# asharakeh/bayes-od-rc

Hardware: AMD Instinct MI355X
Metric: images/sec at N=10 MC samples, 512x512; per-anchor covariance latency (higher is better)
Workload: dtype bf16; 1 GPU; ResNet-50 RetinaNet + covar head, N=10 MC-dropout, 512x512, full BayesOD pipeline (forward+posterior+soft-NMS+cluster-fuse); global_batch=512, mc_samples=10, anchors=49104, parallelism=one GPU (no exchange; N > 1: image-sharded, one RCCL gather/step), visible_gpus=1, gpu_max_hw_queues=4

## Files before the change

### bayes-od-rc_amd/csrc/conv_igemm.hip

```cpp
#include "kernels.h"
#include "philox.h"
#include <cstdlib>
#include <string>
#include <type_traits>

typedef __attribute__((ext_vector_type(8))) short bf16x8;
typedef __attribute__((ext_vector_type(16))) float f32x16;
typedef __attribute__((ext_vector_type(4))) float f32x4;
typedef __attribute__((ext_vector_type(4))) unsigned int u32x4;
typedef __attribute__((ext_vector_type(8))) _Float16 f16x8;
typedef __attribute__((ext_vector_type(8))) int i32x8;
typedef __attribute__((ext_vector_type(6))) int i32x6;
typedef __attribute__((ext_vector_type(4))) int i32x4;
typedef __attribute__((ext_vector_type(16))) float f32x16v;
__device__ __forceinline__ i32x8 mx_cat(const bf16x8& p0, const bf16x8& p1) {
    return __builtin_shufflevector(__builtin_bit_cast(i32x4, p0), __builtin_bit_cast(i32x4, p1), 0, 1, 2, 3, 4, 5, 6, 7);
}

#define GLOBAL_PTR(p) ((const __attribute__((address_space(1))) void*)(p))
#define LDS_PTR(p) ((__attribute__((address_space(3))) void*)(p))

__device__ __forceinline__ float bf16_to_f32(uint32_t v) { return __uint_as_float(v << 16); }
__device__ __forceinline__ uint32_t f32_to_bf16(float f) {
    uint32_t u = __float_as_uint(f);
// ... 2201 lines not shown
                uint4 r;
                r.x = relu_bf16x2(v.x); r.y = relu_bf16x2(v.y); r.z = relu_bf16x2(v.z); r.w = relu_bf16x2(v.w);
                *reinterpret_cast<uint4*>(reinterpret_cast<uint16_t*>(G.out_relu) + e) = r;
            }
        }
        phase_stamp<ABL>(tstamp, 5);
        if constexpr (ABL == 90) { if (threadIdx.x == 0) atomicAdd(&g_phase_cycles[14], __builtin_amdgcn_s_memrealtime() - treal); }
        if (n + 1 < fan) __syncthreads();
    }
}

template <int BC, int BP, int WC, int WP, int ABL, bool XR, bool SPLIT = false>
__global__ __launch_bounds__(64 * WC * WP, (ABL == 10 ? (BC == 64 ? 3 : 2) : 1)) void conv_igemm_kernel(const ConvArgs a) {
    extern __shared__ __attribute__((aligned(16))) char smem[];
    int bx = blockIdx.x, by = blockIdx.y, gz = blockIdx.z;
    const int ny_tiles = a.cout_pad / BC;
    if (!XR && gridDim.y == 1 && ny_tiles > 1) {
        const int nx = (a.M + BP - 1) / BP, q = nx >> 3, r = nx & 7, xcd = bx & 7, slot = bx >> 3;
        const int pj = slot / ny_tiles;
        by = slot - pj * ny_tiles;
        if (pj >= q + (xcd < r ? 1 : 0)) return;
        bx = (xcd < r ? xcd * (q + 1) : r * (q + 1) + (xcd - r) * q) + pj;
    } else {
        const int nb = gridDim.x, q = nb >> 3, r = nb & 7, xcd = bx & 7, idx = bx >> 3;
        bx = (xcd < r ? xcd * (q + 1) : r * (q + 1) + (xcd - r) * q) + idx;
    }
    if (gridDim.z == 1 && a.groups > 1 && a.ksplit <= 1) {
        if (a.fan_chunk > 0) {
            const int nxt = (a.M + BP - 1) / BP, T = a.fan_chunk, per = T * a.groups;
            const int c = bx / per, w = bx - c * per, here = min(T, nxt - c * T);
// ... 305 lines not shown
    ConvArgs a_local = a_in;
    if ((a_local.flags & CONV_DROPOUT) && a_local.drop_threshold == 0) a_local.flags &= ~CONV_DROPOUT;
    static const bool res_register = getenv("BOD_RES_REGISTER") && atoi(getenv("BOD_RES_REGISTER")) == 1;
    if (res_register && a_local.variant == 0 && !a_local.xreuse && !a_local.split && a_local.ksplit <= 1) a_local.variant = 82;
    static const int nt_stores = getenv("BOD_NT_STORES") ? atoi(getenv("BOD_NT_STORES")) : 4;
    if (!(a_local.flags & CONV_OUT_F32) && !a_local.split && a_local.ksplit <= 1 &&
        (((nt_stores & 1) && !a_local.xreuse) || ((nt_stores & 2) && a_local.xreuse) || ((nt_stores & 4) && a_local.xreuse && a_local.fan_count > 1)))
        a_local.flags |= CONV_NT_OUT;
    if (a_local.mx && (((nt_stores & 8) && a_local.fan_count <= 1) || ((nt_stores & 16) && a_local.fan_count > 1))) a_local.flags |= CONV_NT_OUT;
    {
        static const int fan_chunk = getenv("BOD_FAN_CHUNK") ? atoi(getenv("BOD_FAN_CHUNK")) : 16;
        a_local.fan_chunk = (a_local.fan_count > 1 && a_local.groups > 1 && !a_local.mx && !a_local.split) ? fan_chunk : 0;
    }
    const ConvArgs& a = a_local;
    if (a.M <= 0) return hipSuccess;
    if (a.cin % 64 != 0 || a.cout_pad % 64 != 0) return hipErrorInvalidValue;
    if (a.mx) {
        if ((a.mx < 1 || a.mx > 3) || !a.split || a.xreuse != 2 || a.cout_pad != 256 || a.cin != 512 || a.taps != 9 || a.KW != 3 || !a.ext || a.M % 256 != 0 ||
            (a.flags & CONV_OUT_F32) || a.ksplit > 1 || (a.variant != 0 && a.variant != 90 && a.variant != 91) || a.groups < 1 || a.groups > 3)
            return hipErrorInvalidValue;
        for (int g = 0; g < a.groups; ++g)
            if (a.g[g].res || a.g[g].out_relu || a.g[g].ch_w2 || a.g[g].ch_w3 || (a.g[g].w2 && (a.g[g].out_hx || a.fan_count > 1))) return hipErrorInvalidValue;
#ifndef BOD_DEV_MX_ONLY
        if (a.variant == 90 && a.mx == 1) return launch_mx<11>(a, s);
        if (a.variant == 91 && a.mx == 1) return launch_mx<12>(a, s);
#endif
#ifdef BOD_DEV_MX_ONLY
        return a.mx == 1 ? launch_mx<1>(a, s) : hipErrorInvalidValue;
#else
        if (a.mx == 3) return a.variant == 0 ? launch_mx<3>(a, s) : hipErrorInvalidValue;
// ... 40 lines not shown
    }
    if (a.split) {
        if (a.xreuse) {
            if (!(big && a.cout_pad == 256 && a.taps == 9 && a.KW == 3 && a.ext && a.M % 256 == 0) || (a.flags & CONV_OUT_F32)) return hipErrorInvalidValue;
            return launch_cfg<256, 256, 2, 4, 0, true, true>(a, s);
        }
        if (big) return launch_cfg<256, 256, 2, 4, 0, false, true>(a, s);
        if (a.cout_pad % 128 == 0) return launch_cfg<128, 128, 2, 2, 0, false, true>(a, s);
        return launch_cfg<64, 128, 1, 4, 0, false, true>(a, s);
    }
    const int variant = a.variant;
    if (a.xreuse) {
        if (!(big && a.cout_pad == 256 && a.taps == 9 && a.KW == 3 && a.ext && a.M % 256 == 0)) return hipErrorInvalidValue;
        for (int g = 0; g < a.groups; ++g) if (a.g[g].res || a.g[g].out_relu) return hipErrorInvalidValue;
        if (a.flags & CONV_OUT_F32) return hipErrorInvalidValue;
        if (a.xreuse != 2 || a.variant == 81) return launch_cfg<256, 256, 2, 4, 81, true>(a, s);
        if (a.variant == 1) return launch_cfg<256, 256, 2, 4, 1, true>(a, s);
        if (a.variant == 2) return launch_cfg<256, 256, 2, 4, 2, true>(a, s);
        if (a.variant == 4) return launch_cfg<256, 256, 2, 4, 4, true>(a, s);
        if (a.variant == 30) return launch_cfg<256, 256, 2, 4, 30, true>(a, s);
        if (a.variant == 90) return launch_cfg<256, 256, 2, 4, 90, true>(a, s);
        if (a.variant == 96) return launch_xr_persistent<0>(a, s);
        if (a.variant == 31) return launch_cfg<256, 256, 2, 4, 31, true>(a, s);
        if (a.variant != 0 && a.variant != 83) return hipErrorInvalidValue;
        if (a.fan_count > 1) return launch_cfg<256, 256, 2, 4, 5, true>(a, s);
        if (a.plane_h > 0 && !(a.flags & CONV_DROPOUT) && a.variant == 0) return launch_cfg<256, 256, 2, 4, 6, true>(a, s);
        static const bool old_loop = getenv("BOD_TOWER_MIDBAR") && atoi(getenv("BOD_TOWER_MIDBAR")) == 0;
        if (old_loop && a.variant == 0) return launch_cfg<256, 256, 2, 4, 9, true>(a, s);
        return launch_cfg<256, 256, 2, 4, 0, true>(a, s);
    }
// ... 21 lines not shown
```

### bayes-od-rc_amd/csrc/engine.hip

```cpp
#include "../../include/bayesod.h"
#include "kernels.h"

#include <algorithm>
#include <atomic>
#include <cmath>
#include <condition_variable>
#include <deque>
#include <functional>
#include <mutex>
#include <thread>
#include <tuple>
#include <cstdarg>
#include <cstdio>
#include <cstring>
#include <map>
#include <memory>
#include <string>
#include <vector>
#include <dlfcn.h>

namespace {

constexpr float BN_EPS = 1e-3f;

thread_local std::string g_create_error;

struct HostTensor { std::vector<int64_t> shape; std::vector<float> data; };

struct Plane {
    char* d = nullptr;
    int64_t base = 0;
    int64_t bstride = 0;
    int h = 0, w = 0, C = 0, pitch = 0;
};

struct PackedConv { char* w = nullptr; float* bias = nullptr; int cout = 0, cout_pad = 0, taps = 0, kw = 0, cin = 0; };

struct Op {
    enum Kind { STEM, POOL, CONV } kind;
    ConvArgs conv;
    bool is_head3x3 = false;
    double flops = 0;
    std::string name;
    std::string wname[3], bnname[3];
    bool same_geom = false;
    int flavour = 0;
    int head[3] = {-1, -1, -1};
    bool hx_pyramid = false;
};
enum { FLAVOUR_BOTH = 0, FLAVOUR_RAW = 1, FLAVOUR_AGG = 2 };

uint16_t f2bf(float f) {
    uint32_t u; std::memcpy(&u, &f, 4);
    u += 0x7FFFu + ((u >> 16) & 1u);
// ... 185 lines not shown
    char* stem_out = nullptr;
    int es = 2;
    bool split = false;
    char* pyr_hx = nullptr;
    int pyr_fmt = 1;
    int plan_mx = 0;
    int mx = 0;
    Plane pyramid;
    char* head_act[3][2] = {{nullptr}};
    char* head_act_t[3][4] = {{nullptr}};
    float* raw[3] = {nullptr};
    float* agg[3] = {nullptr};
    bool agg_plan = false;
    bool plan_fused_out = false, plan_xreuse = false, plan_xreuse0 = false;
    bool raw_valid = false, agg_valid = false;
    uint64_t last_seed = 0; uint32_t last_first_image = 0;
    std::map<std::string, RowEnt*> tables;
    struct XrTable { RowEnt* rows = nullptr; int2* ext = nullptr; int m = 0; };
    std::map<std::string, XrTable> xr_tables;
    std::vector<Op> ops;
    const float* cur_images = nullptr;

    float* d_anchors = nullptr;
    PostBuffers pb{};
    float* nms_scores = nullptr; int32_t* nms_begin = nullptr;
    int32_t* nms_sel_s[2] = {nullptr, nullptr}; int32_t* nms_nsel_s[2] = {nullptr, nullptr};
    float* out_scores_s[2] = {nullptr, nullptr}; float* out_means_s[2] = {nullptr, nullptr};
    float* out_covs_s[2] = {nullptr, nullptr}; float* out_counts_s[2] = {nullptr, nullptr};
    int32_t* nms_sel = nullptr; int32_t* nms_nsel = nullptr;
    float* out_scores = nullptr; float* out_means = nullptr; float* out_covs = nullptr; float* out_counts = nullptr;
// ... 625 lines not shown
        if (rc == 1) return h->fail(BOD_ERR_INVALID_ARG, "aggregated tiling: no pixel fits a tile (N = %d)", N);
        if (rc == 2) return h->fail(BOD_ERR_INVALID_ARG, "aggregated tiling: extended rows out of order");
        m2a = (int)tiled.size();
        BODCHK(h->dalloc(&d2a, tiled.size(), false));
        BODCHK(h->dalloc(&dexta, ext.size(), false));
        HIPCHK(h, hipMemcpyAsync(d2a, tiled.data(), tiled.size() * sizeof(RowEnt), hipMemcpyHostToDevice, h->stream));
        HIPCHK(h, hipMemcpyAsync(dexta, ext.data(), ext.size() * sizeof(int2), hipMemcpyHostToDevice, h->stream));
        HIPCHK(h, hipStreamSynchronize(h->stream));
        const size_t BA = (size_t)B * h->A;
        BODCHK(h->dalloc(&h->agg[0], BA * c.num_classes));
        BODCHK(h->dalloc(&h->agg[1], BA * 16));
        if (c.has_covar_head) BODCHK(h->dalloc(&h->agg[2], BA * 10));
    } else {
        BODCHK(ensure_raw(h));
    }
    h->agg_plan = agg; h->plan_fused_out = fuse_out; h->plan_xreuse = xreuse; h->plan_xreuse0 = xreuse0; h->plan_mx = mx_plan ? mxf : 0;
    int hfmt[3] = {mxf, mxf, mxf};
    if (mxf == 2) { const char* e = getenv("BOD_MX4_BOX_HX"); if (e && atoi(e) != 0) hfmt[1] = 1; }
    if (mxf == 1) { static const bool cls_h4 = [] { const char* e = getenv("BOD_MX_CLS_H4"); return !e || atoi(e) != 0; }(); if (cls_h4) hfmt[0] = 2; }
    const bool mixed = mx_plan && hfmt[0] != hfmt[1];
    const int pyr_fmt = mixed ? 1 : mxf;
    h->pyr_fmt = pyr_fmt;
    for (int layer = 0; layer < 4; ++layer)
    for (int fpass = 0; fpass < 2; ++fpass)
    for (int part = 0; part < 2; ++part)
    for (int flav = (agg && layer >= 2) ? FLAVOUR_RAW : FLAVOUR_BOTH; flav <= ((agg && layer >= 2) ? FLAVOUR_AGG : FLAVOUR_BOTH); ++flav) {
        static const bool split_on = [] { const char* e = getenv("BOD_SPLIT_AGG_LAUNCH"); return !e || atoi(e) != 0; }();
        const bool split_launch = agg && layer >= 2 && split_on;
        if (fpass == 1 && (!mixed || layer == 0)) continue;
        const int lfmt = !mx_plan ? 0 : layer == 0 ? pyr_fmt : mixed ? (fpass == 0 ? 2 : 1) : mxf;
        if (!split_launch && part == 1) continue;
        if (split_launch && part == 0 && flav == FLAVOUR_AGG) continue;
        const bool both = split_launch && part == 0;
        Op op; op.kind = Op::CONV; op.is_head3x3 = true; op.flavour = both ? FLAVOUR_BOTH : flav;
        int g = 0; PackedConv pc0{};
        double fused_flops = 0;
        for (int hd = 0; hd < nheads; ++hd) {
            if (layer >= kHeadConvs[hd]) continue;
            if (split_launch && (part == 1) != (layer == kHeadConvs[hd] - 1)) continue;
            if (mixed && layer > 0 && hfmt[hd] != lfmt) continue;
            PackedConv pc;
            BODCHK(pack_conv(h, std::string(kHeadPrefix[hd]) + "_" + std::to_string(layer), "", 128, &pc, (mx_plan && (layer > 0 || mx_l0)) ? lfmt : 0));
// ... 8 lines not shown
            cg.out_hx = (mx_plan && layer < kHeadConvs[hd] - 1) ? hfmt[hd] : 0;
            if (fuse_out && layer == kHeadConvs[hd] - 1) {
                PackedConv po;
                BODCHK(pack_conv(h, kHeadPrefix[hd], "", 32, &po));
                if (po.cin != 256 || po.cout != out_ch[hd] || po.taps != 1)
                    return h->fail(BOD_ERR_INVALID_ARG, "head output conv %s must be 1x1 256->%d (got %d->%d)", kHeadPrefix[hd], out_ch[hd], po.cin, po.cout);
                cg.w2 = po.w; cg.bias2 = po.bias; cg.out2 = h->raw[hd]; cg.cout2 = po.cout; cg.out2_cstride = out_ch[hd];
                op.head[g] = hd;
                if (flav == FLAVOUR_AGG) {
                    cg.out2 = nullptr;
                    cg.agg_kind = hd == 0 ? AGG_CLS : hd == 1 ? AGG_BOX : AGG_COV;
                    cg.agg_n = N; cg.agg_P = h->P; cg.agg_C = c.num_classes; cg.agg_out = h->agg[hd]; cg.anchors = h->d_anchors;
                }
                fused_flops += 2.0 * ((double)B * N * h->P) * 256.0 * out_ch[hd];
            }
            op.conv.g[g] = cg;
            if (g == 0) pc0 = pc;
            ++g;
        }
        if (g == 0) continue;
        const int M = layer == 0 ? B * h->P : B * N * h->P;
        ConvArgs a = base_args(pc0, layer == 0 ? d1 : d2, M, 256, 256);
        for (int q = 0; q < g; ++q) a.g[q] = op.conv.g[q];
        a.groups = g;
        a.flags = CONV_RELU | (mc ? CONV_DROPOUT : 0);
        a.fan_count = layer == 0 ? N : 1;
        a.fan_stride = (int32_t)h->Ppad;
        a.drop_threshold = thr; a.drop_scale = dscale;
        a.mx = mx_plan ? ((layer == 0 && !mx_l0) ? 2 : (lfmt == 2 ? 3 : 1)) : 0;
        op.hx_pyramid = mx_l0 && layer == 0;
// ... 2 lines not shown
            static const int tower_loader = getenv("BOD_TOWER_LOADER") ? atoi(getenv("BOD_TOWER_LOADER")) : 0;
            a.mx_loader = mx_plan ? mx_loader : ((h->es == 2 && layer > 0) ? tower_loader : 0);
        }
        if (xreuse0 && layer == 0) { a.rows = d1x; a.M = m1x; a.ext = dext1; a.xreuse = 2; }
        if (xreuse && layer > 0) {
            a.rows = d2x; a.M = m2x; a.ext = dext;
            if (agg && layer >= 2 && !(split_launch && part == 0)) { a.rows = d2a; a.M = m2a; a.ext = dexta; }
            a.xreuse = 2;
        }
        op.conv = a;
        op.flops = 2.0 * M * 256.0 * 2304.0 * g + fused_flops;
        op.name = "head_tower_layer_" + std::to_string(layer) + (both ? "" : flav == FLAVOUR_AGG ? "(aggregating)" : flav == FLAVOUR_RAW ? "(raw)" : "");
        op.same_geom = N == 1;
        h->ops.push_back(op);
    }
    for (int hd = 0; hd < nheads && !fuse_out; ++hd) {
        PackedConv pc;
        BODCHK(pack_conv(h, kHeadPrefix[hd], "", 64, &pc));
        if (pc.cin != 256 || pc.cout != out_ch[hd] || pc.taps != 1)
            return h->fail(BOD_ERR_INVALID_ARG, "head output conv %s must be 1x1 256->%d (got %d->%d)", kHeadPrefix[hd], out_ch[hd], pc.cin, pc.cout);
        Op op; op.kind = Op::CONV;
        ConvArgs a = base_args(pc, d3, B * N * h->P, 256, out_ch[hd]);
        a.g[0] = ConvGroup{train_mode ? h->head_act_t[hd][kHeadConvs[hd] - 1] : h->head_act[hd][(kHeadConvs[hd] - 1) & 1], pc.w, pc.bias, h->raw[hd], nullptr, nullptr, 0, 0, nullptr, nullptr, nullptr, 0, 0};
        a.flags = CONV_OUT_F32;
        op.conv = a;
        op.flops = 2.0 * a.M * pc.cout * 256.0;
        op.name = kHeadPrefix[hd]; op.wname[0] = kHeadPrefix[hd];
        h->ops.push_back(op);
    }
    if (h->splitk_elems) {
// ... 125 lines not shown
    h->ov_dirty = false;
    return BOD_OK;
}

bod_status run_forward(bod_context* h, const float* dev_images, uint64_t seed, uint32_t first_image, int flavour = FLAVOUR_RAW,
                       bool only_flavoured = false, bool overlapped = false) {
    const bod_config& c = h->cfg;
    if (flavour == FLAVOUR_RAW && !only_flavoured) BODCHK(ensure_raw(h));
    const bool ov = overlapped && h->overlap_mode != 0 && !only_flavoured;
    hipStream_t fs = ov ? h->front : h->stream;
    int par = 0;
    if (ov) {
        par = h->fwd_parity; h->fwd_parity ^= 1;
        if (h->l0_pending[par]) { HIPCHK(h, hipStreamWaitEvent(fs, h->ev_l0_done[par], 0)); h->l0_pending[par] = false; }
    }
    if (!only_flavoured) h->pyr_last = par;
    const int cus_front = h->n_cu;
    const int cus_back = h->n_cu;
    static const int trace_call = getenv("BOD_TRACE_OPS") ? atoi(getenv("BOD_TRACE_OPS")) : 0;
    static int call_no = 0;
    const bool trace = trace_call > 0 && ++call_no == trace_call && !ov;
    std::vector<hipEvent_t> tev;
    if (trace) {
        tev.resize(h->ops.size() + 1);
        for (hipEvent_t& e : tev) HIPCHK(h, hipEventCreate(&e));
        HIPCHK(h, hipEventRecord(tev[0], h->stream));
    }
    size_t op_i = 0;
    bool stem_pool_fused = false;
    std::string cur_stage;
    struct StageCloser { std::string& s; ~StageCloser() { if (!s.empty()) markers().pop(); } } stage_closer{cur_stage};
// ... 18 lines not shown
            }
        }
        switch (op.kind) {
            case Op::STEM: {
                const Op* pool = op_i < h->ops.size() && h->ops[op_i].kind == Op::POOL ? &h->ops[op_i] : nullptr;
                static const bool split_fused = [] { const char* e = getenv("BOD_STEM_SPLIT_FUSED"); return !e || atoi(e) != 0; }();
                stem_pool_fused = pool && !h->train && (h->split ? split_fused : h->es == 2) && !trace &&
                                  stem_pool_fused_applies(dev_images, c.batch, c.image_w, h->sw, is_front ? cus_front : cus_back);
                if (stem_pool_fused)
                    HIPCHK(h, launch_stem_pool_fused(dev_images, h->stem_w, h->stem_b, pool->conv.g[0].out, h->split ? 1 : 0, c.batch, c.image_h,
                                                     c.image_w, h->sh, h->sw, h->ph, h->pw, h->pw + 2, (h->ph + 2) * (h->pw + 2), st));
                else
                HIPCHK(h, launch_stem_conv(dev_images, h->stem_w, h->stem_b, h->stem_out, h->es == 4, c.batch, c.image_h,
                                           c.image_w, h->sh, h->sw, st));
                if (!h->train) BODCHK(mark_images_consumed(h, st));
                break;
            }
            case Op::POOL:
                if (stem_pool_fused) break;
                HIPCHK(h, launch_stem_pool(h->stem_out, op.conv.g[0].out, h->split ? 2 : (h->es == 4 ? 1 : 0), c.batch,
                                           h->sh, h->sw, h->ph, h->pw, h->pw + 2, (h->ph + 2) * (h->pw + 2), st));
                break;
            case Op::CONV: {
                if (op.hx_pyramid) HIPCHK(h, launch_pairs_to_hx(h->pyramid.d, h->pyr_hx, (long)c.batch * h->Ppad, 256, st, h->pyr_fmt));
                op.conv.seed_lo = (uint32_t)seed; op.conv.seed_hi = (uint32_t)(seed >> 32);
                op.conv.image_base = first_image;
                op.conv.sample_base = (uint32_t)c.mc_sample_base;
                op.conv.dyn_rng = train_dyn_rng(h);
                const bool is_tower = op.conv.xreuse != 0 && op.conv.fan_count <= 1;
                const bool timed = h->profiling && op.is_head3x3 && (h->prof_which == 0 || (h->prof_which == 1) == is_tower);
// ... 32 lines not shown
    if (trace) {
        HIPCHK(h, hipEventRecord(tev[h->ops.size()], h->stream));
        HIPCHK(h, hipStreamSynchronize(h->stream));
        fprintf(stderr, "# op trace: name kind M taps cin cout_pad groups fan ms TFLOP/s\n");
        for (size_t i = 0; i < h->ops.size(); ++i) {
            float ms = 0.f;
            HIPCHK(h, hipEventElapsedTime(&ms, tev[i], tev[i + 1]));
            const Op& o = h->ops[i];
            fprintf(stderr, "%-28s %d %8d %2d %5d %5d %d %2d %9.4f %8.1f\n", o.name.c_str(), (int)o.kind, o.conv.M, o.conv.taps,
                    o.conv.cin, o.conv.cout_pad, o.conv.groups, o.conv.fan_count, ms, o.flops / (ms * 1e-3) / 1e12);
        }
        for (hipEvent_t& e : tev) hipEventDestroy(e);
    }
    h->forward_done = true; h->posterior_done = h->nms_done = h->cluster_done = false; h->affinity_img = -1;
    h->last_seed = seed; h->last_first_image = first_image;
    if (flavour == FLAVOUR_AGG) { h->agg_valid = true; h->raw_valid = false; }
    else { h->raw_valid = true; if (!only_flavoured) h->agg_valid = false; }
    return BOD_OK;
}

bod_status materialise_raw(bod_context* h) {
    if (h->raw_valid || !h->agg_valid) { BODCHK(ensure_raw(h)); return BOD_OK; }
    BODCHK(ensure_raw(h));
    const bool prof = h->profiling;
    h->profiling = false;
    const bool fd = h->forward_done, pd = h->posterior_done, nd = h->nms_done, cd = h->cluster_done;
    const int aff = h->affinity_img;
    const bod_status st = run_forward(h, h->cur_images, h->last_seed, h->last_first_image, FLAVOUR_RAW, true);
    h->profiling = prof;
    h->forward_done = fd; h->posterior_done = pd; h->nms_done = nd; h->cluster_done = cd; h->affinity_img = aff;
    return st;
}

bod_status run_posterior(bod_context* h, uint64_t seed, uint32_t first_image) {
    if (!h->anchors_ready) return h->fail(BOD_ERR_NOT_READY, "bod_set_anchors has not been called");
    for (int sidx = 0; sidx < 2; ++sidx)
        if (h->side_pending[sidx]) HIPCHK(h, hipStreamWaitEvent(h->stream, h->ev_done[sidx], 0));
    MarkerRange mr("bod:posterior");
    PostCfg pc = post_cfg(h, seed, first_image);
    PostBuffers pb = h->pb;
    pb.cls = h->raw[0]; pb.box = h->raw[1]; pb.cov = h->raw[2]; pb.anchors = h->d_anchors;
    pc.aggregated = (h->agg_valid && !h->raw_valid) ? 1 : 0;
    pb.agg_cls = h->agg[0]; pb.agg_box = h->agg[1]; pb.agg_cov = h->agg[2];
    hipEvent_t e0 = nullptr, e1 = nullptr;
    if (h->profiling) {
        HIPCHK(h, hipEventCreate(&e0)); HIPCHK(h, hipEventCreate(&e1));
        HIPCHK(h, hipEventRecord(e0, h->stream));
    }
    HIPCHK(h, launch_posterior(pc, pb, h->stream));
    if (h->cfg.ranking_method == BOD_RANK_JOINT_ENTROPY && h->cfg.gaussian_isotropic && h->cfg.dirichlet_non_informative)
        HIPCHK(h, launch_joint_entropy_rank(pc, pb, h->stream));
    if (h->profiling) { HIPCHK(h, hipEventRecord(e1, h->stream)); h->ev_post.emplace_back(e0, e1); }
    h->posterior_done = true; h->nms_done = h->cluster_done = false; h->affinity_img = -1;
    return BOD_OK;
}

bod_status run_nms(bod_context* h, hipStream_t st) {
    MarkerRange mr("bod:nms");
    const bod_config& c = h->cfg;
    NmsArgs a{};
    a.B = c.batch; a.A = h->A; a.num_kept = h->pb.num_kept; a.corners = h->pb.corners; a.ranking = h->pb.ranking;
    a.work_scores = h->nms_scores; a.work_begin = h->nms_begin; a.selected = h->nms_sel; a.num_selected = h->nms_nsel;
    a.max_out = c.nms_max_output_size; a.iou_thr = c.nms_iou_threshold; a.sigma = c.nms_soft_sigma; a.variant = c.nms_variant;
    HIPCHK(h, launch_nms(a, st));
// ... 1267 lines not shown
    if (!(rank == root && gathered_host) && slot >= 0) {
        HIPCHK(h, hipEventRecord(h->ev_done[slot], st));
    }
    if (gathered_device) *gathered_device = recv;
    return BOD_OK;
}

bod_status bod_plan_info(bod_handle h, int32_t* info8) {
    if (!h || !info8) return BOD_ERR_INVALID_ARG;
    if (!h->weights_ready) return h->fail(BOD_ERR_NOT_READY, "bod_plan_info: the plan is built by bod_finalize_weights");
    for (int i = 0; i < 8; ++i) info8[i] = 0;
    info8[0] = h->agg_plan; info8[1] = h->plan_fused_out; info8[2] = h->plan_xreuse; info8[3] = h->plan_xreuse0;
    info8[4] = (int32_t)h->ops.size();
    for (const Op& o : h->ops) if (o.kind == Op::CONV && !o.is_head3x3 && o.conv.xreuse) ++info8[5];
    info8[6] = h->plan_mx;
    return BOD_OK;
}

bod_status bod_profile_select(bod_handle h, int32_t which) {
    if (!h) return BOD_ERR_INVALID_ARG;
    if (which < 0 || which > 2) return h->fail(BOD_ERR_INVALID_ARG, "bod_profile_select: %d", which);
    h->prof_which = which;
    return BOD_OK;
}

bod_status bod_profile_end(bod_handle h, double* head_ms, int64_t* head_launches, double* head_flops, double* post_ms, int64_t* post_launches) {
    if (!h) return BOD_ERR_INVALID_ARG;
    BODCHK(join_overlap(h));
    HIPCHK(h, hipStreamSynchronize(h->stream));
    double hm = 0, pm = 0;
// ... 15 lines not shown
```

### bayes-od-rc_amd/csrc/kernels.h

```cpp
#pragma once
#include <hip/hip_runtime.h>
#include <stdint.h>
#include "plan_tables.h"


struct ConvGroup {
    const void* in;
    const void* w;
    const float* bias;
    void* out;
    const void* res;
    void* out_relu;
    int32_t in_coff;
    int32_t layer_id;
    const void* w2;
    const float* bias2;
    float* out2;
    int32_t cout2;
    int32_t out2_cstride;
    int32_t agg_kind;
    int32_t agg_n;
    int32_t agg_P;
    int32_t agg_C;
    float* agg_out;
// ... 30 lines not shown
    int32_t groups;
    int32_t variant;
    const int2* ext;
    int32_t xreuse;
    int32_t ksplit;
    float* partial;
    const uint32_t* dyn_rng;
    uint32_t sample_base;
    int32_t split;
    int32_t plane_h, plane_w;
    int32_t n_cu;
    int32_t stagger_ticks;
    int32_t fan_chunk;
    int32_t mx;
    int32_t mx_loader;
};

struct PerDeviceOnce {
    bool done[64] = {false};
    bool* slot() { int d = 0; if (hipGetDevice(&d) != hipSuccess || d < 0 || d >= 64) d = 0; return &done[d]; }
};

int device_cu_count();
inline int launch_cus(const ConvArgs& a) { return a.n_cu > 0 ? a.n_cu : device_cu_count(); }
hipError_t launch_conv_igemm(const ConvArgs& a, hipStream_t s);
bool conv_igemm_uses_full_cout_tile(const ConvArgs& a);
bool conv_igemm_uses_big_tile(const ConvArgs& a);
void conv_igemm_phase_cycles(unsigned long long* out16, bool reset);
hipError_t launch_conv_igemm_f32(const ConvArgs& a, hipStream_t s);
hipError_t launch_pairs_to_hx(const void* in, void* out, long npix, int C, hipStream_t s, int fmt = 1);
// ... 25 lines not shown
    const float* agg_cov;
    uint8_t* keep;
    float* d_counts;
    int32_t* block_counts;
    int32_t* num_kept;
    float* counts;
    float* score;
    float* means;
    float* covs;
    float* ranking;
    float* corners;
    int32_t* anchor_index;
};

hipError_t launch_posterior(const PostCfg& c, const PostBuffers& b, hipStream_t s);
hipError_t launch_joint_entropy_rank(const PostCfg& c, const PostBuffers& b, hipStream_t s);
hipError_t launch_validation_post(const PostCfg& c, const PostBuffers& b, hipStream_t s);

struct NmsArgs {
    int32_t B, A;
    const int32_t* num_kept;
    const float* corners;
    const float* ranking;
    float* work_scores;
    int32_t* work_begin;
    int32_t* selected;
    int32_t* num_selected;
    int32_t max_out;
    float iou_thr, sigma;
    int32_t variant;
// ... 112 lines not shown
```

### bayes-od-rc_amd/csrc/post_kernels.hip

```cpp
#include "kernels.h"
#include "philox.h"
#include <algorithm>
#include <math.h>

#define POST_BLOCK 256
#define MAXC 16

struct Mat4 { float m[4][4]; };

__device__ __forceinline__ Mat4 inv_spd4_once(const Mat4& a) {
    float g[4][4];
#pragma unroll
    for (int i = 0; i < 4; ++i)
#pragma unroll
        for (int j = 0; j < 4; ++j) g[i][j] = 0.f;
#pragma unroll
    for (int j = 0; j < 4; ++j) {
        float d = a.m[j][j];
#pragma unroll
        for (int k = 0; k < j; ++k) d -= g[j][k] * g[j][k];
        const float dj = sqrtf(d);
        g[j][j] = dj;
        const float inv = 1.0f / dj;
#pragma unroll
// ... 444 lines not shown
}
#if defined(BOD_POST_SELFCHECK)
extern "C" int bod_debug_selfcheck_read(unsigned int* count, unsigned long long* waves, void* recs, int max) {
    unsigned int n = 0;
    if (hipMemcpyFromSymbol(&n, HIP_SYMBOL(g_selfcheck_count), 4) != hipSuccess) return 1;
    if (hipMemcpyFromSymbol(waves, HIP_SYMBOL(g_selfcheck_waves), 8) != hipSuccess) return 1;
    const unsigned int m = n < (unsigned)max ? n : (unsigned)max;
    if (m && hipMemcpyFromSymbol(recs, HIP_SYMBOL(g_selfcheck_recs), (size_t)(m < 4096u ? m : 4096u) * sizeof(SelfcheckRec)) != hipSuccess) return 1;
    const unsigned int z = 0; const unsigned long long z8 = 0;
    if (hipMemcpyToSymbol(HIP_SYMBOL(g_selfcheck_count), &z, 4) != hipSuccess || hipMemcpyToSymbol(HIP_SYMBOL(g_selfcheck_waves), &z8, 8) != hipSuccess) return 1;
    *count = n;
    return 0;
}
#endif

hipError_t launch_posterior(const PostCfg& c, const PostBuffers& b, hipStream_t s) {
    const int nblocks = (c.A + POST_BLOCK - 1) / POST_BLOCK;
    dim3 grid(nblocks, c.B);
    if (c.C == 8) {
        hipLaunchKernelGGL(post_sample_kernel<8>, grid, dim3(POST_BLOCK), 0, s, c, b, nblocks);
        hipLaunchKernelGGL(post_scan_kernel, dim3(c.B), dim3(POST_BLOCK), 0, s, b, nblocks);
        hipLaunchKernelGGL(post_compact_kernel, grid, dim3(POST_BLOCK), 0, s, c, b, nblocks);
        hipLaunchKernelGGL(post_fuse_kernel<8>, dim3(std::min(nblocks, POST_FUSE_BLOCKS), c.B), dim3(POST_BLOCK), 0, s, c, b, nblocks);
    } else if (c.C == 4) {
        hipLaunchKernelGGL(post_sample_kernel<4>, grid, dim3(POST_BLOCK), 0, s, c, b, nblocks);
        hipLaunchKernelGGL(post_scan_kernel, dim3(c.B), dim3(POST_BLOCK), 0, s, b, nblocks);
        hipLaunchKernelGGL(post_compact_kernel, grid, dim3(POST_BLOCK), 0, s, c, b, nblocks);
        hipLaunchKernelGGL(post_fuse_kernel<4>, dim3(std::min(nblocks, POST_FUSE_BLOCKS), c.B), dim3(POST_BLOCK), 0, s, c, b, nblocks);
    } else {
        return hipErrorInvalidValue;
    }
    return hipGetLastError();
}

template <int C>
__global__ __launch_bounds__(POST_BLOCK) void val_flag_kernel(PostCfg c, PostBuffers pb, int nblocks) {
    const int a = blockIdx.x * POST_BLOCK + threadIdx.x;
    const int b = blockIdx.y;
    bool keep = false;
    if (a < c.A) {
        const float* l = pb.cls + (((size_t)b * c.N) * c.A + a) * C;
        float v[C];
#pragma unroll
        for (int j = 0; j < C; ++j) v[j] = l[j];
        float mx = v[0];
#pragma unroll
// ... 570 lines not shown
```

### bayes-od-rc_amd/engine.py

```python
import ctypes as C

import numpy as np

from . import _lib
from ._lib import BodConfig, BodSizes, as_f32, fptr, iptr

_KINDS = {"kernel": 0, "bias": 1, "gamma": 2, "beta": 3, "mean": 4, "var": 5}
PRECISIONS = {"bf16": 0, "fp32": 1, "bf16x3": 2, "f16mx": 3, "f16mx4": 4}


def make_config(image_hw, batch=1, mc_samples=10, num_classes=8, anchors_per_location=9, device=0,
                dropout_rate=0.3, use_full_covar=True, bayes_od_config=None, nms_config=None,
                has_covar_head=True, dataset_name='bdd', orig_size=None, nms_variant='A',
                num_categorical_draws=30, layers=(3, 4, 5, 6, 7), precision='bf16', mc_sample_base=0,
                mc_ensemble_size=0, training=False, backbone_depth=50, pipeline_overlap=False):
    bo = bayes_od_config or {'ranking_method': 'score', 'dirichlet_prior': {'type': 'non_informative'},
                             'gaussian_prior': {'type': 'isotropic', 'isotropic_variance': 100000.0}}
    nms = nms_config or {'max_output_size': 100, 'iou_threshold': 0.5, 'soft_nms_sigma': 0.5}
    cfg = BodConfig()
    cfg.device = int(device)
    cfg.image_h, cfg.image_w = int(image_hw[0]), int(image_hw[1])
    cfg.batch, cfg.mc_samples = int(batch), int(mc_samples)
    cfg.num_classes = int(num_classes)
    cfg.anchors_per_location = int(anchors_per_location)
# ... 343 lines not shown
        out = None
        dev = C.c_void_p(0)
        if rank == root and want_host:
            out = np.empty((world, self.B, self.K, w), np.float32)
        self._chk(self.lib.bod_gather_detections(self.h, int(slot), C.c_void_p(int(comm) if comm else 0), int(world), int(rank), int(root),
                                                 out.ctypes.data if out is not None else None,
                                                 C.byref(dev) if rank == root else None))
        if rank == root and not want_host:
            return int(dev.value or 0), (world, self.B, self.K, w)
        return out

    def plan_info(self):
        info = (C.c_int32 * 8)()
        self._chk(self.lib.bod_plan_info(self.h, info))
        return {"aggregating": bool(info[0]), "fused_head_outputs": bool(info[1]), "row_reuse": bool(info[2]),
                "fan_out_row_reuse": bool(info[3]), "ops": int(info[4]), "plane_row_reuse_layers": int(info[5]), "tower_mx": bool(info[6]), "tower_mx_format": int(info[6])}

    @property
    def aggregating(self):
        return self.plan_info()["aggregating"]

    def profile_begin(self, which=None):
        if which is not None:
            self._chk(self.lib.bod_profile_select(self.h, int(which)))
        self._chk(self.lib.bod_profile_begin(self.h))

    def profile_end(self):
        hm, pm, fl = C.c_double(0), C.c_double(0), C.c_double(0)
        hl, pl = C.c_int64(0), C.c_int64(0)
        self._chk(self.lib.bod_profile_end(self.h, C.byref(hm), C.byref(hl), C.byref(fl), C.byref(pm), C.byref(pl)))
        return {"head_conv_ms": hm.value, "head_conv_launches": hl.value, "head_conv_flops": fl.value,
# ... 46 lines not shown
```

Baseline: 1916 images/sec.

## Compute box/covariance head tower tail only at pixels kept by class posterior

Splits the posterior into a keep stage and a fuse stage. After the class head runs, a keep-mask kernel builds a compact list of tiles holding only the pixels that have surviving anchors. The last tower layer and the output convs of the box and covariance heads then run only on those tiles via a device-side tile count. This avoids computing box and covariance heads for anchors the class filter discards. The cost is an extra single-threaded-per-image tile builder, extra buffers, and a fallback that rematerialises the raw outputs when the seed or image changes.

```diff
diff --git a/bayes-od-rc_amd/csrc/conv_igemm.hip b/bayes-od-rc_amd/csrc/conv_igemm.hip
--- a/bayes-od-rc_amd/csrc/conv_igemm.hip
+++ b/bayes-od-rc_amd/csrc/conv_igemm.hip
@@ -2239,6 +2239,13 @@
 __global__ __launch_bounds__(64 * WC * WP, (ABL == 10 ? (BC == 64 ? 3 : 2) : 1)) void conv_igemm_kernel(const ConvArgs a) {
     extern __shared__ __attribute__((aligned(16))) char smem[];
     int bx = blockIdx.x, by = blockIdx.y, gz = blockIdx.z;
+    if constexpr (XR) {
+        if (a.tile_count) {
+            if (bx >= *a.tile_count) return;
+            conv_tile<BC, BP, WC, WP, ABL, XR, SPLIT>(a, gz, bx, by, smem);
+            return;
+        }
+    }
     const int ny_tiles = a.cout_pad / BC;
     if (!XR && gridDim.y == 1 && ny_tiles > 1) {
         const int nx = (a.M + BP - 1) / BP, q = nx >> 3, r = nx & 7, xcd = bx & 7, slot = bx >> 3;
@@ -2574,6 +2581,7 @@
     }
     const ConvArgs& a = a_local;
     if (a.M <= 0) return hipSuccess;
+    if (a.tile_count && (a.mx || a.split || !a.xreuse || a.ksplit > 1)) return hipErrorInvalidValue;
     if (a.cin % 64 != 0 || a.cout_pad % 64 != 0) return hipErrorInvalidValue;
     if (a.mx) {
         if ((a.mx < 1 || a.mx > 3) || !a.split || a.xreuse != 2 || a.cout_pad != 256 || a.cin != 512 || a.taps != 9 || a.KW != 3 || !a.ext || a.M % 256 != 0 ||
@@ -2644,6 +2652,7 @@
         if (!(big && a.cout_pad == 256 && a.taps == 9 && a.KW == 3 && a.ext && a.M % 256 == 0)) return hipErrorInvalidValue;
         for (int g = 0; g < a.groups; ++g) if (a.g[g].res || a.g[g].out_relu) return hipErrorInvalidValue;
         if (a.flags & CONV_OUT_F32) return hipErrorInvalidValue;
+        if (a.tile_count) return (a.xreuse == 2 && a.variant == 0 && a.fan_count <= 1) ? launch_cfg<256, 256, 2, 4, 0, true>(a, s) : hipErrorInvalidValue;
         if (a.xreuse != 2 || a.variant == 81) return launch_cfg<256, 256, 2, 4, 81, true>(a, s);
         if (a.variant == 1) return launch_cfg<256, 256, 2, 4, 1, true>(a, s);
         if (a.variant == 2) return launch_cfg<256, 256, 2, 4, 2, true>(a, s);
diff --git a/bayes-od-rc_amd/csrc/engine.hip b/bayes-od-rc_amd/csrc/engine.hip
--- a/bayes-od-rc_amd/csrc/engine.hip
+++ b/bayes-od-rc_amd/csrc/engine.hip
@@ -37,7 +37,7 @@
 struct PackedConv { char* w = nullptr; float* bias = nullptr; int cout = 0, cout_pad = 0, taps = 0, kw = 0, cin = 0; };
 
 struct Op {
-    enum Kind { STEM, POOL, CONV } kind;
+    enum Kind { STEM, POOL, CONV, KEEP } kind;
     ConvArgs conv;
     bool is_head3x3 = false;
     double flops = 0;
@@ -253,6 +253,11 @@
     bool agg_plan = false;
     bool plan_fused_out = false, plan_xreuse = false, plan_xreuse0 = false;
     bool raw_valid = false, agg_valid = false;
+    bool plan_sparse = false;
+    SparseTailArgs sparse{};
+    bool agg_sparse = false;
+    bool keep_ready = false;
+    uint64_t keep_seed = 0; uint32_t keep_first = 0;
     uint64_t last_seed = 0; uint32_t last_first_image = 0;
     std::map<std::string, RowEnt*> tables;
     struct XrTable { RowEnt* rows = nullptr; int2* ext = nullptr; int m = 0; };
@@ -908,6 +913,28 @@
     } else {
         BODCHK(ensure_raw(h));
     }
+    static const bool split_on = [] { const char* e = getenv("BOD_SPLIT_AGG_LAUNCH"); return !e || atoi(e) != 0; }();
+    bool sparse = agg && split_on && h->es == 2 && !h->split && !mx_plan && !c.pipeline_overlap && h->A == h->P * c.anchors_per_location &&
+                  h->P <= 65536;
+    if (const char* e = getenv("BOD_SPARSE_TAIL")) sparse = sparse && atoi(e) != 0;
+    if (sparse) {
+        SparseTailArgs& sa = h->sparse;
+        sa.B = B; sa.N = N; sa.P = h->P; sa.apl = c.anchors_per_location; sa.Ppad = h->Ppad;
+        sa.cap_tiles = B * (h->P / sparse_tail_min_pixels(N) + 1);
+        RowEnt* pix = nullptr;
+        BODCHK(h->dalloc(&pix, (size_t)h->P, false));
+        HIPCHK(h, hipMemcpyAsync(pix, t2.data(), (size_t)h->P * sizeof(RowEnt), hipMemcpyHostToDevice, h->stream));
+        HIPCHK(h, hipStreamSynchronize(h->stream));
+        sa.pix = pix;
+        BODCHK(h->dalloc(&sa.rows, (size_t)sa.cap_tiles * 256, false));
+        BODCHK(h->dalloc(&sa.ext, (size_t)sa.cap_tiles * XR_EXT_ROWS, false));
+        BODCHK(h->dalloc(&sa.tile_count, 1));
+        BODCHK(h->dalloc(&sa.chunks, (size_t)B * h->P, false));
+        BODCHK(h->dalloc(&sa.tiles, (size_t)B * h->P, false));
+    }
+    h->plan_sparse = sparse;
+    Op sparse_op; sparse_op.kind = Op::CONV; sparse_op.is_head3x3 = true; sparse_op.flavour = FLAVOUR_AGG;
+    int sparse_groups = 0; PackedConv sparse_pc{};
     h->agg_plan = agg; h->plan_fused_out = fuse_out; h->plan_xreuse = xreuse; h->plan_xreuse0 = xreuse0; h->plan_mx = mx_plan ? mxf : 0;
     int hfmt[3] = {mxf, mxf, mxf};
     if (mxf == 2) { const char* e = getenv("BOD_MX4_BOX_HX"); if (e && atoi(e) != 0) hfmt[1] = 1; }
@@ -919,7 +946,6 @@
     for (int fpass = 0; fpass < 2; ++fpass)
     for (int part = 0; part < 2; ++part)
     for (int flav = (agg && layer >= 2) ? FLAVOUR_RAW : FLAVOUR_BOTH; flav <= ((agg && layer >= 2) ? FLAVOUR_AGG : FLAVOUR_BOTH); ++flav) {
-        static const bool split_on = [] { const char* e = getenv("BOD_SPLIT_AGG_LAUNCH"); return !e || atoi(e) != 0; }();
         const bool split_launch = agg && layer >= 2 && split_on;
         if (fpass == 1 && (!mixed || layer == 0)) continue;
         const int lfmt = !mx_plan ? 0 : layer == 0 ? pyr_fmt : mixed ? (fpass == 0 ? 2 : 1) : mxf;
@@ -958,6 +984,16 @@
                 }
                 fused_flops += 2.0 * ((double)B * N * h->P) * 256.0 * out_ch[hd];
             }
+            if (sparse && flav == FLAVOUR_AGG && hd != 0) {
+                sparse_op.conv.g[sparse_groups] = cg;
+                sparse_op.wname[sparse_groups] = op.wname[g];
+                sparse_op.head[sparse_groups] = hd;
+                if (sparse_groups++ == 0) sparse_pc = pc;
+                sparse_op.flops += 2.0 * ((double)B * N * h->P) * 256.0 * 2304.0 + 2.0 * ((double)B * N * h->P) * 256.0 * out_ch[hd];
+                fused_flops -= 2.0 * ((double)B * N * h->P) * 256.0 * out_ch[hd];
+                op.head[g] = -1; op.wname[g].clear();
+                continue;
+            }
             op.conv.g[g] = cg;
             if (g == 0) pc0 = pc;
             ++g;
@@ -990,6 +1026,22 @@
         op.same_geom = N == 1;
         h->ops.push_back(op);
     }
+    if (sparse_groups > 0) {
+        Op keep; keep.kind = Op::KEEP; keep.flavour = FLAVOUR_AGG; keep.name = "head_tower_layer_3(keep)";
+        h->ops.push_back(keep);
+        const SparseTailArgs& sa = h->sparse;
+        ConvArgs a = base_args(sparse_pc, sa.rows, sa.cap_tiles * 256, 256, 256);
+        for (int q = 0; q < sparse_groups; ++q) a.g[q] = sparse_op.conv.g[q];
+        a.groups = sparse_groups;
+        a.flags = CONV_RELU | (mc ? CONV_DROPOUT : 0);
+        a.fan_count = 1; a.fan_stride = (int32_t)h->Ppad;
+        a.drop_threshold = thr; a.drop_scale = dscale;
+        a.ext = sa.ext; a.xreuse = 2; a.tile_count = sa.tile_count;
+        a.mx_loader = getenv("BOD_TOWER_LOADER") ? atoi(getenv("BOD_TOWER_LOADER")) : 0;
+        sparse_op.conv = a;
+        sparse_op.name = "head_tower_layer_3(sparse)";
+        h->ops.push_back(sparse_op);
+    }
     for (int hd = 0; hd < nheads && !fuse_out; ++hd) {
         PackedConv pc;
         BODCHK(pack_conv(h, kHeadPrefix[hd], "", 64, &pc));
@@ -1145,7 +1197,7 @@
         par = h->fwd_parity; h->fwd_parity ^= 1;
         if (h->l0_pending[par]) { HIPCHK(h, hipStreamWaitEvent(fs, h->ev_l0_done[par], 0)); h->l0_pending[par] = false; }
     }
-    if (!only_flavoured) h->pyr_last = par;
+    if (!only_flavoured) { h->pyr_last = par; h->keep_ready = false; }
     const int cus_front = h->n_cu;
     const int cus_back = h->n_cu;
     static const int trace_call = getenv("BOD_TRACE_OPS") ? atoi(getenv("BOD_TRACE_OPS")) : 0;
@@ -1194,6 +1246,20 @@
                 HIPCHK(h, launch_stem_conv(dev_images, h->stem_w, h->stem_b, h->stem_out, h->es == 4, c.batch, c.image_h,
                                            c.image_w, h->sh, h->sw, st));
                 if (!h->train) BODCHK(mark_images_consumed(h, st));
+                break;
+            }
+            case Op::KEEP: {
+                for (int sidx = 0; sidx < 2; ++sidx)
+                    if (h->side_pending[sidx]) HIPCHK(h, hipStreamWaitEvent(st, h->ev_done[sidx], 0));
+                PostCfg pc = post_cfg(h, seed, first_image);
+                pc.aggregated = 1;
+                PostBuffers pb = h->pb;
+                pb.agg_cls = h->agg[0];
+                HIPCHK(h, launch_posterior_keep(pc, pb, st));
+                SparseTailArgs sa = h->sparse;
+                sa.keep = h->pb.keep;
+                HIPCHK(h, launch_sparse_tail_rows(sa, st));
+                h->keep_ready = true; h->keep_seed = seed; h->keep_first = first_image;
                 break;
             }
             case Op::POOL:
@@ -1256,7 +1322,7 @@
     }
     h->forward_done = true; h->posterior_done = h->nms_done = h->cluster_done = false; h->affinity_img = -1;
     h->last_seed = seed; h->last_first_image = first_image;
-    if (flavour == FLAVOUR_AGG) { h->agg_valid = true; h->raw_valid = false; }
+    if (flavour == FLAVOUR_AGG) { h->agg_valid = true; h->raw_valid = false; h->agg_sparse = h->plan_sparse; }
     else { h->raw_valid = true; if (!only_flavoured) h->agg_valid = false; }
     return BOD_OK;
 }
@@ -1284,12 +1350,19 @@
     pb.cls = h->raw[0]; pb.box = h->raw[1]; pb.cov = h->raw[2]; pb.anchors = h->d_anchors;
     pc.aggregated = (h->agg_valid && !h->raw_valid) ? 1 : 0;
     pb.agg_cls = h->agg[0]; pb.agg_box = h->agg[1]; pb.agg_cov = h->agg[2];
+    const bool keep_done = pc.aggregated && h->keep_ready && seed == h->keep_seed && first_image == h->keep_first;
+    h->keep_ready = false;
+    if (pc.aggregated && h->agg_sparse && (seed != h->keep_seed || first_image != h->keep_first)) {
+        BODCHK(materialise_raw(h));
+        pc.aggregated = 0;
+        pb.cls = h->raw[0]; pb.box = h->raw[1]; pb.cov = h->raw[2];
+    }
     hipEvent_t e0 = nullptr, e1 = nullptr;
     if (h->profiling) {
         HIPCHK(h, hipEventCreate(&e0)); HIPCHK(h, hipEventCreate(&e1));
         HIPCHK(h, hipEventRecord(e0, h->stream));
     }
-    HIPCHK(h, launch_posterior(pc, pb, h->stream));
+    HIPCHK(h, keep_done ? launch_posterior_fuse(pc, pb, h->stream) : launch_posterior(pc, pb, h->stream));
     if (h->cfg.ranking_method == BOD_RANK_JOINT_ENTROPY && h->cfg.gaussian_isotropic && h->cfg.dirichlet_non_informative)
         HIPCHK(h, launch_joint_entropy_rank(pc, pb, h->stream));
     if (h->profiling) { HIPCHK(h, hipEventRecord(e1, h->stream)); h->ev_post.emplace_back(e0, e1); }
@@ -2587,6 +2660,7 @@
     info8[4] = (int32_t)h->ops.size();
     for (const Op& o : h->ops) if (o.kind == Op::CONV && !o.is_head3x3 && o.conv.xreuse) ++info8[5];
     info8[6] = h->plan_mx;
+    info8[7] = h->plan_sparse;
     return BOD_OK;
 }
 
diff --git a/bayes-od-rc_amd/csrc/kernels.h b/bayes-od-rc_amd/csrc/kernels.h
--- a/bayes-od-rc_amd/csrc/kernels.h
+++ b/bayes-od-rc_amd/csrc/kernels.h
@@ -68,6 +68,7 @@
     int32_t fan_chunk;
     int32_t mx;
     int32_t mx_loader;
+    const int32_t* tile_count;
 };
 
 struct PerDeviceOnce {
@@ -123,6 +124,22 @@
 };
 
 hipError_t launch_posterior(const PostCfg& c, const PostBuffers& b, hipStream_t s);
+hipError_t launch_posterior_keep(const PostCfg& c, const PostBuffers& b, hipStream_t s);
+hipError_t launch_posterior_fuse(const PostCfg& c, const PostBuffers& b, hipStream_t s);
+
+struct SparseTailArgs {
+    const uint8_t* keep;
+    const RowEnt* pix;
+    RowEnt* rows;
+    int2* ext;
+    int32_t* tile_count;
+    int4* chunks;
+    int4* tiles;
+    int32_t B, N, P, apl, cap_tiles;
+    int64_t Ppad;
+};
+int sparse_tail_min_pixels(int N);
+hipError_t launch_sparse_tail_rows(const SparseTailArgs& a, hipStream_t s);
 hipError_t launch_joint_entropy_rank(const PostCfg& c, const PostBuffers& b, hipStream_t s);
 hipError_t launch_validation_post(const PostCfg& c, const PostBuffers& b, hipStream_t s);
 
diff --git a/bayes-od-rc_amd/csrc/post_kernels.hip b/bayes-od-rc_amd/csrc/post_kernels.hip
--- a/bayes-od-rc_amd/csrc/post_kernels.hip
+++ b/bayes-od-rc_amd/csrc/post_kernels.hip
@@ -482,22 +482,123 @@
 }
 #endif
 
-hipError_t launch_posterior(const PostCfg& c, const PostBuffers& b, hipStream_t s) {
+hipError_t launch_posterior_keep(const PostCfg& c, const PostBuffers& b, hipStream_t s) {
     const int nblocks = (c.A + POST_BLOCK - 1) / POST_BLOCK;
     dim3 grid(nblocks, c.B);
-    if (c.C == 8) {
-        hipLaunchKernelGGL(post_sample_kernel<8>, grid, dim3(POST_BLOCK), 0, s, c, b, nblocks);
-        hipLaunchKernelGGL(post_scan_kernel, dim3(c.B), dim3(POST_BLOCK), 0, s, b, nblocks);
-        hipLaunchKernelGGL(post_compact_kernel, grid, dim3(POST_BLOCK), 0, s, c, b, nblocks);
-        hipLaunchKernelGGL(post_fuse_kernel<8>, dim3(std::min(nblocks, POST_FUSE_BLOCKS), c.B), dim3(POST_BLOCK), 0, s, c, b, nblocks);
-    } else if (c.C == 4) {
-        hipLaunchKernelGGL(post_sample_kernel<4>, grid, dim3(POST_BLOCK), 0, s, c, b, nblocks);
-        hipLaunchKernelGGL(post_scan_kernel, dim3(c.B), dim3(POST_BLOCK), 0, s, b, nblocks);
-        hipLaunchKernelGGL(post_compact_kernel, grid, dim3(POST_BLOCK), 0, s, c, b, nblocks);
-        hipLaunchKernelGGL(post_fuse_kernel<4>, dim3(std::min(nblocks, POST_FUSE_BLOCKS), c.B), dim3(POST_BLOCK), 0, s, c, b, nblocks);
-    } else {
-        return hipErrorInvalidValue;
-    }
+    if (c.C == 8) hipLaunchKernelGGL(post_sample_kernel<8>, grid, dim3(POST_BLOCK), 0, s, c, b, nblocks);
+    else if (c.C == 4) hipLaunchKernelGGL(post_sample_kernel<4>, grid, dim3(POST_BLOCK), 0, s, c, b, nblocks);
+    else return hipErrorInvalidValue;
+    hipLaunchKernelGGL(post_scan_kernel, dim3(c.B), dim3(POST_BLOCK), 0, s, b, nblocks);
+    return hipGetLastError();
+}
+
+hipError_t launch_posterior_fuse(const PostCfg& c, const PostBuffers& b, hipStream_t s) {
+    const int nblocks = (c.A + POST_BLOCK - 1) / POST_BLOCK;
+    dim3 grid(nblocks, c.B);
+    if (c.C != 8 && c.C != 4) return hipErrorInvalidValue;
+    hipLaunchKernelGGL(post_compact_kernel, grid, dim3(POST_BLOCK), 0, s, c, b, nblocks);
+    if (c.C == 8) hipLaunchKernelGGL(post_fuse_kernel<8>, dim3(std::min(nblocks, POST_FUSE_BLOCKS), c.B), dim3(POST_BLOCK), 0, s, c, b, nblocks);
+    else hipLaunchKernelGGL(post_fuse_kernel<4>, dim3(std::min(nblocks, POST_FUSE_BLOCKS), c.B), dim3(POST_BLOCK), 0, s, c, b, nblocks);
+    return hipGetLastError();
+}
+
+hipError_t launch_posterior(const PostCfg& c, const PostBuffers& b, hipStream_t s) {
+    const hipError_t e = launch_posterior_keep(c, b, s);
+    return e != hipSuccess ? e : launch_posterior_fuse(c, b, s);
+}
+
+int sparse_tail_min_pixels(int N) {
+    const int Qmax = 256 / N;
+    return std::max(1, std::min(Qmax, (XR_EXT_ROWS - 3 * N) / (3 * N) + 1));
+}
+
+__device__ __forceinline__ RowEnt sparse_tail_ent(const SparseTailArgs& a, int b, int n, int p) {
+    RowEnt e = a.pix[p];
+    const int32_t plane = (int32_t)(((int64_t)b * a.N + n) * a.Ppad);
+    e.in_off += plane;
+    e.out_off += plane;
+    e.rng_zs = n | (b << 16);
+    e.pad0 = (int32_t)(((int64_t)b * a.N + n) * a.P + p);
+    return e;
+}
+
+__global__ __launch_bounds__(256) void sparse_tail_rows_kernel(SparseTailArgs a) {
+    extern __shared__ uint8_t s_flag[];
+    __shared__ int s_nchunk, s_ntile, s_base;
+    const int b = blockIdx.x, tid = threadIdx.x, N = a.N, P = a.P;
+    const uint8_t* keep = a.keep + (size_t)b * P * a.apl;
+    for (int p = tid; p < P; p += blockDim.x) {
+        uint8_t f = 0;
+        for (int k = 0; k < a.apl; ++k) f |= keep[(size_t)p * a.apl + k];
+        s_flag[p] = f ? 1 : 0;
+    }
+    __syncthreads();
+    int4* chunks = a.chunks + (size_t)b * P;
+    int4* tiles = a.tiles + (size_t)b * P;
+    if (tid == 0) {
+        const int Qmax = 256 / N;
+        auto adjacent = [&](int p) { return a.pix[p].in_off == a.pix[p - 1].in_off + 1 && a.pix[p].in_pitch == a.pix[p - 1].in_pitch; };
+        int nchunk = 0, ntile = 0, Q = 0, X = 0, first = 0;
+        bool open = false;
+        auto close_tile = [&]() { tiles[ntile++] = make_int4(first, Q, X, 0); open = false; };
+        int p = 0;
+        while (p < P) {
+            if (!s_flag[p]) { ++p; continue; }
+            int L = 1;
+            while (p + L < P && adjacent(p + L) &&
+                   (s_flag[p + L] || (p + L + 1 < P && s_flag[p + L + 1] && adjacent(p + L + 1)))) ++L;
+            while (L > 0) {
+                if (!open) { first = p; Q = 0; X = 0; open = true; }
+                const int take = min(min(L, Qmax - Q), (XR_EXT_ROWS - X) / N - 2);
+                if (take < 1) { close_tile(); continue; }
+                chunks[nchunk++] = make_int4(p, ntile, Q, X | (take << 16));
+                X += N * (take + 2); Q += take; p += take; L -= take;
+                if (Q == Qmax) close_tile();
+            }
+        }
+        if (open) close_tile();
+        s_nchunk = nchunk; s_ntile = ntile;
+        s_base = atomicAdd(a.tile_count, ntile);
+    }
+    __syncthreads();
+    const int nchunk = s_nchunk, ntile = s_ntile, base = s_base;
+    if (base + ntile > a.cap_tiles) return;
+    for (int i = tid; i < nchunk * N; i += blockDim.x) {
+        const int ci = i / N, n = i - ci * N;
+        const int4 c = chunks[ci];
+        const int p0 = c.x, t = base + c.y, Q0 = c.z, X0 = c.w & 0xFFFF, take = c.w >> 16;
+        const int x0 = X0 + n * (take + 2);
+        const RowEnt first = sparse_tail_ent(a, b, n, p0);
+        int2* ext = a.ext + (size_t)t * XR_EXT_ROWS + x0;
+        for (int k = 0; k < take + 2; ++k) ext[k] = make_int2(first.in_off + k, first.in_pitch);
+        RowEnt* rows = a.rows + (size_t)t * 256;
+        for (int k = 0; k < take; ++k) {
+            RowEnt q = sparse_tail_ent(a, b, n, p0 + k);
+            q.pad1 = x0 + k;
+            rows[(Q0 + k) * N + n] = q;
+        }
+    }
+    RowEnt invalid = a.pix[0];
+    invalid.out_off = -1; invalid.pad0 = 0; invalid.pad1 = 0;
+    for (int i = tid; i < ntile * 256; i += blockDim.x) {
+        const int t = i >> 8, r = i & 255;
+        if (r >= tiles[t].y * N) a.rows[(size_t)(base + t) * 256 + r] = invalid;
+    }
+    for (int i = tid; i < ntile * XR_EXT_ROWS; i += blockDim.x) {
+        const int t = i / XR_EXT_ROWS, r = i - t * XR_EXT_ROWS;
+        const int4 ti = tiles[t];
+        if (r >= ti.z) {
+            const RowEnt first = sparse_tail_ent(a, b, 0, ti.x);
+            a.ext[(size_t)(base + t) * XR_EXT_ROWS + r] = make_int2(first.in_off, first.in_pitch);
+        }
+    }
+}
+
+hipError_t launch_sparse_tail_rows(const SparseTailArgs& a, hipStream_t s) {
+    if (a.B <= 0 || a.P <= 0 || a.N < 1 || 256 / a.N < 1 || XR_EXT_ROWS / a.N - 2 < 1 || a.P > 65536) return hipErrorInvalidValue;
+    hipError_t e = hipMemsetAsync(a.tile_count, 0, sizeof(int32_t), s);
+    if (e != hipSuccess) return e;
+    hipLaunchKernelGGL(sparse_tail_rows_kernel, dim3(a.B), dim3(256), (size_t)a.P, s, a);
     return hipGetLastError();
 }
 
diff --git a/bayes-od-rc_amd/engine.py b/bayes-od-rc_amd/engine.py
--- a/bayes-od-rc_amd/engine.py
+++ b/bayes-od-rc_amd/engine.py
@@ -381,7 +381,8 @@
         info = (C.c_int32 * 8)()
         self._chk(self.lib.bod_plan_info(self.h, info))
         return {"aggregating": bool(info[0]), "fused_head_outputs": bool(info[1]), "row_reuse": bool(info[2]),
-                "fan_out_row_reuse": bool(info[3]), "ops": int(info[4]), "plane_row_reuse_layers": int(info[5]), "tower_mx": bool(info[6]), "tower_mx_format": int(info[6])}
+                "fan_out_row_reuse": bool(info[3]), "ops": int(info[4]), "plane_row_reuse_layers": int(info[5]), "tower_mx": bool(info[6]), "tower_mx_format": int(info[6]),
+                "sparse_tail": bool(info[7])}
 
     @property
     def aggregating(self):
```

Result: faster. 2173 images/sec (median of 6 runs) (+13.4%).
